# Drexubery/ViewCrafter

Measured on AMD Instinct MI355X. Metric: DDIM steps/sec (576x1024x25f latent 25x72x128, CFG 7.5, 50-step schedule), higher is better.
Workload: dtype f16; 1 GPU; ViewCrafter_25_576x1024x25; trajectories_per_gpu=1, frames=25, parallelism=trajectory-sharded x1 (no in-step collective)

## Files before the change

include/vcx.h:

```cpp
#ifndef VCX_H
#define VCX_H

#include <stddef.h>
#include <stdint.h>

#ifdef __cplusplus
extern "C" {
#endif

#define VCX_OK 0
#define VCX_EINVAL (-1)
#define VCX_ELAUNCH (-2)
#define VCX_ENODEV (-3)

#define VCX_ABI_VERSION 14

int vcx_abi_version(void);
const char* vcx_last_error(void);
int vcx_device_arch(char* name_host, int len);

#define VCX_GEMM_BIAS_N 0x1
#define VCX_GEMM_BIAS_M 0x2
#define VCX_GEMM_ROWADD 0x4
#define VCX_GEMM_RESIDUAL 0x8
#define VCX_GEMM_GEGLU 0x10
#define VCX_GEMM_OUT_F32 0x20
#define VCX_GEMM_CONV_SLABK 0x40
#define VCX_GEMM_LNFOLD 0x80
#define VCX_GEMM_LNFOLD_T 0x100
#define VCX_GEMM_COLSTATS 0x200
#define VCX_GEMM_ROWSTATS 0x400
#define VCX_GEMM_MXFP8_OUT 0x800

typedef struct vcx_gemm_desc {
    size_t struct_size;
    const void* A;
    const void* W;
    void* C;
    const float* bias;
    const float* rowadd;
    const void* residual;
    int64_t lda;
    int32_t M, N, K;
    int32_t ldw, ldc, ldr;
    int32_t mode;
    int32_t in_h, in_w, out_h, out_w, cin, kh, kw, stride, pad_h, pad_w, ups;
    int32_t rowadd_div;
    int32_t flags;
    float alpha;
    const float* ln_stats;
    const float* ln_colsum;
    float* colstats;
    int64_t ldcs;
    float* rowstats;
    float rowstats_eps;
    int32_t rowadd_ld;
    const void* tail_a0;
    const void* tail_a1;
    int64_t tail_lda0;
    int64_t tail_lda1;
    int32_t tail_k0;
    int32_t tail_k1;
} vcx_gemm_desc;

int vcx_gemm_f16(const vcx_gemm_desc* desc_host, void* stream);
int vcx_gemm_units_f16(const vcx_gemm_desc* desc_host, int unit_rows, int64_t w_unit_stride, int64_t bias_unit_stride, void* stream);

enum {
    VCX_ROUTE_REFUSED = 0,
    VCX_ROUTE_REGISTER = 1,
    VCX_ROUTE_TILED = 2,
    VCX_ROUTE_WS320 = 3,
    VCX_ROUTE_WS320_GEGLU = 4,
    VCX_ROUTE_WS320_LNF = 5,
    VCX_ROUTE_UNITS_WS320 = 6,
    VCX_ROUTE_UNITS_GROUPED = 7,
    VCX_ROUTE_UNITS_LOOP = 8
};
int vcx_gemm_route(const vcx_gemm_desc* desc_host, int unit_rows);

size_t vcx_groupnorm_ws_bytes(int n_outer, int64_t pixels, int groups);
int vcx_groupnorm_stats_f16(const void* x, float* stats, void* ws, int n_outer, int64_t pixels,
                            int C, int groups, void* stream);
int vcx_groupnorm_apply_f16(const void* x, void* y, const float* stats, const float* gamma,
                            const float* beta, int n_outer, int64_t pixels, int C, int groups,
                            float eps, int silu, void* stream);
int vcx_groupnorm_apply2_f16(const void* x1, int c1, const void* x2, void* y, const float* stats, const float* gamma, const float* beta,
                             int n_outer, int64_t pixels, int C, int groups, float eps, int silu, void* stream);
int vcx_groupnorm_stats_from_colstats_f32(const float* colstats, float* stats, void* ws, int n_outer, int64_t pixels, int C,
                                          int groups, void* stream);

int vcx_groupnorm_fold_linear_f16(const float* W, const float* bias, const float* gamma, const float* beta, const float* stats,
                                  void* Wn, float* bn, int n_outer, int N, int C, int groups, float eps, void* stream);

int vcx_rowstats_f16(const void* x, float* stats, int64_t rows, int C, float eps, void* stream);
int vcx_layernorm_f16(const void* x, void* y, const float* gamma, const float* beta,
                      int64_t rows, int C, float eps, void* stream);

int vcx_quant_mxfp8_f16(const void* x, int64_t ldx, void* q, void* scales, int64_t rows, int K, void* stream);
int vcx_layernorm_mxfp8_f16(const void* x, void* q, void* scales, const float* gamma, const float* beta, int64_t rows, int C, float eps,
                            void* stream);
int vcx_gemm_mxfp8(const void* a, const void* a_scales, const void* w, const void* w_scales, void* out, void* out_scales, const float* bias,
                   const void* residual, int64_t M, int64_t N, int64_t K, int64_t ldc, int64_t ldr, int flags, void* stream);
int vcx_gemm_mxfp8_ok(int64_t M, int64_t N, int64_t K, int flags);
int vcx_groupnorm_apply_mxfp8_f16(const void* x, void* q, void* scales, const float* stats, const float* gamma, const float* beta, int n_outer,
                                  int64_t pixels, int C, int groups, float eps, int silu, void* stream);
int vcx_conv_t3_mxfp8(const void* a, const void* a_scales, const void* w, const void* w_scales, void* out, const float* bias, const void* residual,
                      float* colstats, int64_t B, int64_t T, int64_t P, int64_t Cin, int64_t N, int64_t ldc, int64_t ldr, int64_t ldcs, int flags,
                      void* stream);
int vcx_conv_t3_mxfp8_ok(int64_t B, int64_t T, int64_t P, int64_t Cin, int64_t N, int64_t ldc, int64_t ldr, int64_t ldcs, int64_t colstats_col,
                         int flags);
int vcx_groupnorm_apply2_mxfp8_f16(const void* x1, int c1, const void* x2, void* q, void* scales, const float* stats, const float* gamma,
                                   const float* beta, int n_outer, int64_t pixels, int C, int groups, float eps, int silu, void* stream);
int vcx_conv3x3_mxfp8(const void* a, const void* a_scales, const void* w, const void* w_scales, void* out, const float* bias, const float* rowadd,
                      const void* residual, float* colstats, int64_t n, int64_t H, int64_t W, int64_t Cin, int64_t N, int64_t ldc, int64_t ldr,
                      int64_t ldcs, int64_t rowadd_ld, int64_t rowadd_div, int flags, void* stream);
int vcx_conv3x3_mxfp8_ok(int64_t n, int64_t H, int64_t W, int64_t Cin, int64_t N, int64_t ldc, int64_t ldr, int64_t ldcs, int64_t colstats_col,
                         int64_t rowadd_div, int flags);

#define VCX_ATTN_ACCUMULATE 1
#define VCX_ATTN_LOG2_LOGITS 2
int vcx_attn_flash_d64_f16(const void* q, const void* k, const void* vt, void* o, int n_groups,
                           int heads, int nq, int nk, int kv_rows, int kv_div, int64_t ldq,
                           int64_t ldk, int64_t ldvt, int64_t ldo, float scale, int flags,
                           void* stream);

int vcx_attn_flash_dual_d64_f16(const void* q, const void* k1, const void* vt1, const void* k2,
                                const void* vt2, void* o, int n_groups, int heads, int nq,
                                int nk1, int kv_rows1, int kv_div1, int64_t ldk1, int64_t ldvt1,
                                int nk2, int kv_rows2, int kv_div2, int64_t ldk2, int64_t ldvt2,
                                int64_t ldq, int64_t ldo, float scale, int flags, void* stream);

int vcx_attn_flash_d512_f16(const void* q, const void* k, const void* vt, void* o, int n_groups, int nq, int nk, int kv_rows,
                            int64_t ldq, int64_t ldk, int64_t ldvt, int64_t ldo, float scale, void* stream);

int vcx_attn_temporal_d64_f16(const void* qkv, void* o, int B, int T, int64_t P, int heads,
                              int64_t ld, int k_off, int v_off, int64_t ldo, float scale,
                              void* stream);
#define VCX_ATTN_CAUSAL 4
int vcx_attn_temporal_d64_masked_f16(const void* qkv, void* o, int B, int T, int64_t P, int heads,
                                     int64_t ld, int k_off, int v_off, int64_t ldo, float scale,
                                     int flags, void* stream);
int vcx_attn_temporal_d64_rel_f16(const void* qkv, void* o, const void* relg, void* relp, int R, int B, int T, int64_t P,
                                  int heads, int64_t ld, int k_off, int v_off, int64_t ldo, float scale, int flags,
                                  void* stream);

int vcx_softmax_rows_f16(void* x, int64_t rows, int n, int64_t ld, void* stream);

int vcx_silu_f32(const float* x, float* y, int64_t n, void* stream);
int vcx_gelu_f16(const void* x, void* y, int64_t n, void* stream);
int vcx_clip_preprocess_f32(const float* x, float* y, int B, int C, int H, int W, int size, int antialias,
                            const float* mean_host, const float* std_host, void* stream);
int vcx_timestep_embedding_f32(const int64_t* t, float* out, int B, int dim, float max_period,
                               void* stream);
int vcx_cast_f32_to_f16(const float* x, void* y, int64_t n, void* stream);
int vcx_cast_f16_to_f32(const void* x, float* y, int64_t n, void* stream);
int vcx_copy2d_f16(const void* src, void* dst, int64_t rows, int cols, int64_t lds, int64_t ldd,
                   void* stream);
int vcx_avgpool2x2_f16(const void* x, void* y, int n, int H, int W, int C, void* stream);
int vcx_upsample2x_f16(const void* x, void* y, int n, int H, int W, int C, void* stream);
int vcx_add_nchw_f32_to_nhwc_f16(const float* src, void* h, int n, int C, int64_t HW, void* stream);
int vcx_ncthw_f32_to_nthwc_f16(const float* src, void* dst, int B, int C, int T, int64_t HW,
                               int ldc, int c_off, float scale, void* stream);
int vcx_nthwc_to_ncthw_f32(const void* src, float* dst, int B, int C, int T, int64_t HW, int ldc,
                           int src_f32, void* stream);

size_t vcx_ddim_ws_bytes(int B, int64_t n);
int vcx_ddim_step_f32(const float* x, const float* v_cond, const float* v_uncond,
                      const float* noise, float* x_prev, float* pred_x0, void* ws,
                      size_t ws_bytes, int B, int64_t n, const float* coef_host, void* stream);
int vcx_ddim_step3_f32(const float* x, const float* v_cond, const float* v_uncond,
                       const float* v_img, const float* noise, float* x_prev, float* pred_x0,
                       void* ws, size_t ws_bytes, int B, int64_t n, const float* coef_host,
                       void* stream);

#define VCX_PROF_FAMILIES 6
int vcx_profile_begin(int max_records);
int vcx_profile_end(double* out_host);

#define VCX_TUNE_GEMM_CFG 0
#define VCX_TUNE_GEMM_DMA 1
#define VCX_TUNE_FLASH_QB 2
#define VCX_TUNE_XATTN_RESIDENT 3
#define VCX_TUNE_FLASH_IMPL 4
#define VCX_TUNE_EXP0 5
#define VCX_TUNE_EXP1 6
#define VCX_TUNE_GEMM_WS 7
#define VCX_TUNE_COUNT 8
int vcx_tune_set(int knob, int value);
int vcx_tune_get(int knob);

#ifdef __cplusplus
}
#endif
#endif
```

viewcrafter_amd/_lib.py:

```python
import ctypes
import os
from ctypes import c_char_p, c_double, c_float, c_int, c_int32, c_int64, c_void_p, POINTER

_HERE = os.path.dirname(os.path.abspath(__file__))
LIB_PATH = os.path.join(_HERE, "libvcx.so")

SYMBOLS = [
    "vcx_abi_version", "vcx_last_error", "vcx_device_arch", "vcx_gemm_f16", "vcx_gemm_units_f16", "vcx_gemm_route", "vcx_quant_mxfp8_f16", "vcx_layernorm_mxfp8_f16", "vcx_gemm_mxfp8", "vcx_gemm_mxfp8_ok",
    "vcx_groupnorm_apply_mxfp8_f16", "vcx_conv_t3_mxfp8", "vcx_conv_t3_mxfp8_ok",
    "vcx_groupnorm_apply2_mxfp8_f16", "vcx_conv3x3_mxfp8", "vcx_conv3x3_mxfp8_ok",
    "vcx_groupnorm_ws_bytes", "vcx_groupnorm_stats_f16", "vcx_groupnorm_apply_f16", "vcx_groupnorm_apply2_f16", "vcx_groupnorm_stats_from_colstats_f32", "vcx_groupnorm_fold_linear_f16", "vcx_layernorm_f16", "vcx_rowstats_f16",
    "vcx_attn_flash_d64_f16", "vcx_attn_flash_d512_f16", "vcx_attn_flash_dual_d64_f16", "vcx_attn_temporal_d64_f16", "vcx_attn_temporal_d64_masked_f16", "vcx_attn_temporal_d64_rel_f16", "vcx_softmax_rows_f16",
    "vcx_silu_f32", "vcx_gelu_f16", "vcx_clip_preprocess_f32", "vcx_add_nchw_f32_to_nhwc_f16", "vcx_timestep_embedding_f32", "vcx_cast_f32_to_f16", "vcx_cast_f16_to_f32",
    "vcx_copy2d_f16", "vcx_avgpool2x2_f16", "vcx_upsample2x_f16", "vcx_ncthw_f32_to_nthwc_f16", "vcx_nthwc_to_ncthw_f32", "vcx_ddim_ws_bytes", "vcx_ddim_step_f32", "vcx_ddim_step3_f32",
    "vcx_profile_begin", "vcx_profile_end", "vcx_tune_set", "vcx_tune_get",
]

ABI_VERSION = 14
TUNE = {"GEMM_CFG": (0, -1), "GEMM_DMA": (1, 1), "FLASH_QB": (2, 0), "XATTN_RESIDENT": (3, 1), "FLASH_IMPL": (4, 0), "EXP0": (5, 0),
        "EXP1": (6, 0), "GEMM_WS": (7, 1)}
GEMM_BIAS_N, GEMM_BIAS_M, GEMM_ROWADD, GEMM_RESIDUAL, GEMM_GEGLU, GEMM_OUT_F32, GEMM_CONV_SLABK = 1, 2, 4, 8, 16, 32, 64
GEMM_LNFOLD, GEMM_LNFOLD_T, GEMM_COLSTATS, GEMM_ROWSTATS, GEMM_MXFP8_OUT = 0x80, 0x100, 0x200, 0x400, 0x800
ROUTE_REFUSED, ROUTE_REGISTER, ROUTE_TILED, ROUTE_WS320, ROUTE_WS320_GEGLU, ROUTE_WS320_LNF, ROUTE_UNITS_WS320, ROUTE_UNITS_GROUPED, ROUTE_UNITS_LOOP = range(9)
PROF_FAMILIES = ("gemm", "flash_attn", "temporal_attn", "groupnorm", "layernorm", "elementwise")


class GemmDesc(ctypes.Structure):
    _fields_ = [
        ("struct_size", ctypes.c_size_t),
        ("A", c_void_p), ("W", c_void_p), ("C", c_void_p), ("bias", c_void_p), ("rowadd", c_void_p),
        ("residual", c_void_p), ("lda", c_int64), ("M", c_int32), ("N", c_int32), ("K", c_int32),
        ("ldw", c_int32), ("ldc", c_int32), ("ldr", c_int32), ("mode", c_int32),
        ("in_h", c_int32), ("in_w", c_int32), ("out_h", c_int32), ("out_w", c_int32), ("cin", c_int32),
        ("kh", c_int32), ("kw", c_int32), ("stride", c_int32), ("pad_h", c_int32), ("pad_w", c_int32),
        ("ups", c_int32), ("rowadd_div", c_int32), ("flags", c_int32), ("alpha", c_float),
        ("ln_stats", c_void_p), ("ln_colsum", c_void_p), ("colstats", c_void_p), ("ldcs", c_int64),
        ("rowstats", c_void_p), ("rowstats_eps", c_float), ("rowadd_ld", c_int32),
        ("tail_a0", c_void_p), ("tail_a1", c_void_p), ("tail_lda0", c_int64), ("tail_lda1", c_int64), ("tail_k0", c_int32), ("tail_k1", c_int32),
    ]

    def __init__(self, *args, **kw):
        super().__init__(*args, **kw)
        self.struct_size = ctypes.sizeof(GemmDesc)


_lib = None


class VcxError(RuntimeError):
    pass


def lib():
    global _lib
    if _lib is not None:
        return _lib
    if not os.path.exists(LIB_PATH):
        raise VcxError(
            f"{LIB_PATH} not found: build it with `make -C viewcrafter_amd/csrc` "
            "(or `python -c 'import __graft_entry__ as g; g.build()'`). There is no fallback path.")
    import torch
    L = ctypes.CDLL(LIB_PATH)
    L.vcx_abi_version.restype = c_int
    L.vcx_last_error.restype = c_char_p
    L.vcx_device_arch.argtypes = [c_char_p, c_int]
    L.vcx_gemm_f16.argtypes = [POINTER(GemmDesc), c_void_p]
    L.vcx_gemm_units_f16.argtypes = [POINTER(GemmDesc), c_int, c_int64, c_int64, c_void_p]
    L.vcx_gemm_route.argtypes = [POINTER(GemmDesc), c_int]
    L.vcx_quant_mxfp8_f16.argtypes = [c_void_p, c_int64, c_void_p, c_void_p, c_int64, c_int, c_void_p]
    L.vcx_layernorm_mxfp8_f16.argtypes = [c_void_p, c_void_p, c_void_p, c_void_p, c_void_p, c_int64, c_int, c_float, c_void_p]
    L.vcx_gemm_mxfp8.argtypes = [c_void_p, c_void_p, c_void_p, c_void_p, c_void_p, c_void_p, c_void_p, c_void_p, c_int64, c_int64, c_int64, c_int64,
                                 c_int64, c_int, c_void_p]
    L.vcx_gemm_mxfp8_ok.argtypes = [c_int64, c_int64, c_int64, c_int]
    L.vcx_groupnorm_apply_mxfp8_f16.argtypes = [c_void_p, c_void_p, c_void_p, c_void_p, c_void_p, c_void_p, c_int, c_int64, c_int, c_int, c_float, c_int, c_void_p]
    L.vcx_conv_t3_mxfp8.argtypes = [c_void_p, c_void_p, c_void_p, c_void_p, c_void_p, c_void_p, c_void_p, c_void_p, c_int64, c_int64, c_int64, c_int64, c_int64,
                                    c_int64, c_int64, c_int64, c_int, c_void_p]
    L.vcx_conv_t3_mxfp8_ok.argtypes = [c_int64, c_int64, c_int64, c_int64, c_int64, c_int64, c_int64, c_int64, c_int64, c_int]
    L.vcx_groupnorm_apply2_mxfp8_f16.argtypes = [c_void_p, c_int, c_void_p, c_void_p, c_void_p, c_void_p, c_void_p, c_void_p, c_int, c_int64, c_int, c_int, c_float,
                                                 c_int, c_void_p]
    L.vcx_conv3x3_mxfp8.argtypes = [c_void_p, c_void_p, c_void_p, c_void_p, c_void_p, c_void_p, c_void_p, c_void_p, c_void_p, c_int64, c_int64, c_int64, c_int64,
                                    c_int64, c_int64, c_int64, c_int64, c_int64, c_int64, c_int, c_void_p]
    L.vcx_conv3x3_mxfp8_ok.argtypes = [c_int64, c_int64, c_int64, c_int64, c_int64, c_int64, c_int64, c_int64, c_int64, c_int64, c_int]
    L.vcx_groupnorm_ws_bytes.argtypes = [c_int, c_int64, c_int]
    L.vcx_groupnorm_stats_f16.argtypes = [c_void_p, c_void_p, c_void_p, c_int, c_int64, c_int, c_int, c_void_p]
    L.vcx_groupnorm_apply_f16.argtypes = [c_void_p, c_void_p, c_void_p, c_void_p, c_void_p, c_int, c_int64, c_int,
                                          c_int, c_float, c_int, c_void_p]
    L.vcx_groupnorm_apply2_f16.argtypes = [c_void_p, c_int, c_void_p, c_void_p, c_void_p, c_void_p, c_void_p, c_int, c_int64, c_int,
                                           c_int, c_float, c_int, c_void_p]
    L.vcx_layernorm_f16.argtypes = [c_void_p, c_void_p, c_void_p, c_void_p, c_int64, c_int, c_float, c_void_p]
    L.vcx_rowstats_f16.argtypes = [c_void_p, c_void_p, c_int64, c_int, c_float, c_void_p]
    L.vcx_groupnorm_stats_from_colstats_f32.argtypes = [c_void_p, c_void_p, c_void_p, c_int, c_int64, c_int, c_int, c_void_p]
    L.vcx_groupnorm_fold_linear_f16.argtypes = [c_void_p, c_void_p, c_void_p, c_void_p, c_void_p, c_void_p, c_void_p, c_int, c_int, c_int, c_int,
                                                c_float, c_void_p]
    L.vcx_attn_flash_d64_f16.argtypes = [c_void_p, c_void_p, c_void_p, c_void_p, c_int, c_int, c_int, c_int, c_int,
                                         c_int, c_int64, c_int64, c_int64, c_int64, c_float, c_int, c_void_p]
    L.vcx_attn_flash_d512_f16.argtypes = [c_void_p, c_void_p, c_void_p, c_void_p, c_int, c_int, c_int, c_int, c_int64, c_int64, c_int64, c_int64, c_float, c_void_p]
    L.vcx_attn_flash_dual_d64_f16.argtypes = [c_void_p, c_void_p, c_void_p, c_void_p, c_void_p, c_void_p, c_int, c_int, c_int,
                                              c_int, c_int, c_int, c_int64, c_int64, c_int, c_int, c_int, c_int64, c_int64,
                                              c_int64, c_int64, c_float, c_int, c_void_p]
    L.vcx_attn_temporal_d64_f16.argtypes = [c_void_p, c_void_p, c_int, c_int, c_int64, c_int, c_int64, c_int, c_int,
                                            c_int64, c_float, c_void_p]
    L.vcx_attn_temporal_d64_masked_f16.argtypes = [c_void_p, c_void_p, c_int, c_int, c_int64, c_int, c_int64, c_int, c_int,
                                            c_int64, c_float, c_int, c_void_p]
    L.vcx_attn_temporal_d64_rel_f16.argtypes = [c_void_p, c_void_p, c_void_p, c_void_p, c_int, c_int, c_int, c_int64, c_int, c_int64, c_int, c_int,
                                                c_int64, c_float, c_int, c_void_p]
    L.vcx_softmax_rows_f16.argtypes = [c_void_p, c_int64, c_int, c_int64, c_void_p]
    L.vcx_silu_f32.argtypes = [c_void_p, c_void_p, c_int64, c_void_p]
    L.vcx_gelu_f16.argtypes = [c_void_p, c_void_p, c_int64, c_void_p]
    L.vcx_add_nchw_f32_to_nhwc_f16.argtypes = [c_void_p, c_void_p, c_int, c_int, c_int64, c_void_p]
    L.vcx_clip_preprocess_f32.argtypes = [c_void_p, c_void_p, c_int, c_int, c_int, c_int, c_int, c_int, POINTER(c_float), POINTER(c_float),
                                          c_void_p]
    L.vcx_timestep_embedding_f32.argtypes = [c_void_p, c_void_p, c_int, c_int, c_float, c_void_p]
    L.vcx_cast_f32_to_f16.argtypes = [c_void_p, c_void_p, c_int64, c_void_p]
    L.vcx_cast_f16_to_f32.argtypes = [c_void_p, c_void_p, c_int64, c_void_p]
    L.vcx_copy2d_f16.argtypes = [c_void_p, c_void_p, c_int64, c_int, c_int64, c_int64, c_void_p]
    L.vcx_avgpool2x2_f16.argtypes = [c_void_p, c_void_p, c_int, c_int, c_int, c_int, c_void_p]
    L.vcx_upsample2x_f16.argtypes = [c_void_p, c_void_p, c_int, c_int, c_int, c_int, c_void_p]
    L.vcx_ncthw_f32_to_nthwc_f16.argtypes = [c_void_p, c_void_p, c_int, c_int, c_int, c_int64, c_int, c_int, c_float,
                                             c_void_p]
    L.vcx_nthwc_to_ncthw_f32.argtypes = [c_void_p, c_void_p, c_int, c_int, c_int, c_int64, c_int, c_int, c_void_p]
    L.vcx_ddim_ws_bytes.restype = ctypes.c_size_t
    L.vcx_ddim_ws_bytes.argtypes = [c_int, c_int64]
    L.vcx_ddim_step_f32.argtypes = [c_void_p, c_void_p, c_void_p, c_void_p, c_void_p, c_void_p, c_void_p, ctypes.c_size_t, c_int,
                                    c_int64, POINTER(c_float), c_void_p]
    L.vcx_ddim_step3_f32.argtypes = [c_void_p, c_void_p, c_void_p, c_void_p, c_void_p, c_void_p, c_void_p, c_void_p, ctypes.c_size_t,
                                     c_int, c_int64, POINTER(c_float), c_void_p]
    L.vcx_profile_begin.argtypes = [c_int]
    L.vcx_profile_end.argtypes = [POINTER(c_double)]
    L.vcx_tune_set.argtypes = [c_int, c_int]
    L.vcx_tune_get.argtypes = [c_int]
    for name in SYMBOLS:
        fn = getattr(L, name)
        if name == "vcx_groupnorm_ws_bytes":
            fn.restype = ctypes.c_size_t
        elif name != "vcx_last_error":
            fn.restype = c_int
    if L.vcx_abi_version() != ABI_VERSION:
        raise VcxError(f"libvcx ABI version {L.vcx_abi_version()} != {ABI_VERSION}; rebuild the library (make -C viewcrafter_amd/csrc)")
    _lib = L
    return L


def check(rc, what=""):
    if rc != 0:
        msg = lib().vcx_last_error().decode("utf-8", "replace")
        raise VcxError(f"libvcx call failed ({rc}) {what}: {msg}")
```

viewcrafter_amd/lvdm/modules/networks/openaimodel3d.py:

```python
import os

import torch
from torch import nn

from .... import ops
from ....packing import pack_conv, pack_conv3x3_mxfp8, pack_conv_t3_mxfp8, pack_conv_ups_folded
from ..attention import PackedModule, SpatialTransformer, TemporalTransformer, _f16, _f32
from ..flow import CAT_SPLIT, GN_EPILOGUE_STATS, GN_STATS_LEVEL, CatTarget, Flow, out_kwargs as _out_kwargs

SKIP_FOLD = os.environ.get("VCX_SKIP_FOLD", "1") != "0"
EMB_BATCHED = os.environ.get("VCX_EMB_BATCHED", "1") != "0"
TCONV_MXFP8 = os.environ.get("VCX_TCONV_MXFP8", "0") == "1"
TCONV_MXFP8_SKIP_DIMS = frozenset(int(v) for v in os.environ.get("VCX_TCONV_MXFP8_SKIP_DIMS", "320").split(",") if v.strip())
RESCONV_MXFP8 = os.environ.get("VCX_RESCONV_MXFP8", "0") == "1"
RESCONV_MXFP8_SKIP_DIMS = frozenset(int(v) for v in os.environ.get("VCX_RESCONV_MXFP8_SKIP_DIMS", "").split(",") if v.strip())
RESCONV_MXFP8_KEEP_FOLD = os.environ.get("VCX_RESCONV_MXFP8_KEEP_FOLD", "0") == "1"

class TimestepBlock(nn.Module):
    """Marker: modules whose forward takes the timestep embedding (reference openaimodel3d.py:19-28)."""


class TimestepEmbedSequential(nn.Sequential, TimestepBlock):

    def forward(self, x, emb, context=None, batch_size=None, cfg_repeat=1, flow=None, x2=None):
# ... 587 lines not shown
            h = ops.linear(f_emb, *pk["fe"][0], out_f32=True)
            emb = ops.linear(ops.to_f16(ops.silu_f32(h)), *pk["fe"][1], out_f32=True, rowadd=emb, rowadd_div=1)
        return ops.to_f16(ops.silu_f32(emb))

    def forward(self, x, timesteps, context=None, features_adapter=None, fs=None, **kwargs):
        if self.use_hip_graph and features_adapter is None and torch.cuda.is_available() and not torch.cuda.is_current_stream_capturing():
            return self.forward_graphed(x, timesteps, context, fs, cfg_repeat=int(kwargs.get("cfg_repeat", 1) or 1))
        return self._forward(x, timesteps, context=context, features_adapter=features_adapter, fs=fs, **kwargs)

    def forward_graphed(self, x, timesteps, context, fs, cfg_repeat=1):
        parts = list(x) if isinstance(x, (list, tuple)) else [x]
        key = (tuple(tuple(p.shape) for p in parts), context.data_ptr(), context._version, tuple(context.shape),
               None if fs is None else tuple(fs.shape), cfg_repeat)
        ent = self._graphs.get(key)
        if ent is None:
            static = dict(parts=[p.detach().clone().float() for p in parts], t=timesteps.detach().clone(),
                          fs=None if fs is None else fs.detach().clone())
            with torch.no_grad():
                self._forward(static["parts"], static["t"], context=context, fs=static["fs"], cfg_repeat=cfg_repeat)
                torch.cuda.synchronize()
                graph = torch.cuda.CUDAGraph()
                with torch.cuda.graph(graph):
                    out = self._forward(static["parts"], static["t"], context=context, fs=static["fs"], cfg_repeat=cfg_repeat)
            if len(self._graphs) >= 4:
                self._graphs.clear()
            ent = self._graphs[key] = (graph, static, out, context, self._context_kv(context, static["parts"][0].shape[2]))
        graph, static, out = ent[:3]
        for dst, src in zip(static["parts"], parts):
            dst.copy_(src)
        static["t"].copy_(timesteps)
        if fs is not None:
            static["fs"].copy_(fs)
        graph.replay()
        return out

    def _forward(self, x, timesteps, context=None, features_adapter=None, fs=None, cfg_repeat=1, **kwargs):
        ops.require_gpu()
        parts = list(x) if isinstance(x, (list, tuple)) else [x]
        b, _, t, hh, ww = parts[0].shape
        device = parts[0].device
        cin = sum(p.shape[1] for p in parts)
        if cin != self.in_channels:
            raise ValueError(f"expected {self.in_channels} input channels, got {cin}")
        r = int(cfg_repeat or 1)
        if context.shape[0] != b * r:
            raise ValueError(f"context batch {context.shape[0]} != {b} videos x cfg_repeat {r}")
        pk = self.packed()
        emb = self._embed(pk, timesteps, fs, b, device)
        ckv = self._context_kv(context, t)
        rbs = self.resblocks()
        if EMB_BATCHED and all(o % 4 == 0 for o, _ in pk["emb_off"].values()):
            emb_all = ops.linear(emb, pk["emb_w"], pk["emb_b"], out_f32=True)
            if r > 1:
                n_all = emb_all.shape[1]
                emb_all = ops.repeat_rows(emb_all.view(torch.float16).view(b, 2 * n_all), r).view(torch.float32).view(r * b, n_all)
            for rb in rbs:
                o, n_e = pk["emb_off"][id(rb)]
                rb._emb_all = emb_all[:, o:o + n_e]
        try:
            return self._forward_body(parts, pk, emb, ckv, b, t, hh, ww, cin, r, device, features_adapter)
        finally:
            for rb in rbs:
                rb._emb_all = None

    def _forward_body(self, parts, pk, emb, ckv, b, t, hh, ww, cin, r, device, features_adapter):
        cur_b = b

        def replicate(a):
            n_, H_, W_, C_ = a.shape
            return ops.repeat_rows(a.view(n_ * H_ * W_, C_), r).view(r * n_, H_, W_, C_)

        h = torch.empty((b, t, hh, ww, cin), dtype=torch.float16, device=device)
        off = 0
        for p in parts:
            ops.ncthw_to_nthwc(p.float(), h, c_off=off)
            off += p.shape[1]
        h = h.view(b * t, hh, ww, cin)

        lvl2 = GN_STATS_LEVEL >= 2

        def replicate_cs(c):
            if c is None:
                return None
            strips, C_, _ = c.shape
            return ops.repeat_rows(c.view(torch.float16).view(strips, C_ * 4), r).view(torch.float32).view(r * strips, C_, 2)

        hs = []
        adapter_idx = 0
        cs = None
        for i, module in enumerate(self.input_blocks):
            flow = Flow(colstats=cs, want=lvl2)
            if i == 0:
                h = ops.conv2d(h, pk["w_in"], pk["b_in"], kh=3, kw=3)
                flow.colstats = None
                if self.addition_attention:
                    h = self.init_attn(h, emb, context=ckv, batch_size=cur_b, flow=flow)
            elif cur_b != b * r and any(isinstance(layer, SpatialTransformer) for layer in module):
                h = module(h, emb, context=ckv, batch_size=cur_b, cfg_repeat=r, flow=flow)
                cur_b = b * r
                emb = ops.repeat_rows(emb, r)
                hs = [(replicate(a), replicate_cs(c)) for a, c in hs]
            else:
                h = module(h, emb, context=ckv, batch_size=cur_b, flow=flow)
            cs = flow.colstats
            if features_adapter is not None and (i + 1) % 3 == 0:
                h = ops.add_nchw_(h.contiguous(), _adapter_rows(features_adapter[adapter_idx], h.shape[0]))
                adapter_idx, cs = adapter_idx + 1, None
            hs.append((h, cs))
        if features_adapter is not None and len(features_adapter) != adapter_idx:
            raise ValueError("Wrong features_adapter")
        if cur_b != b * r:
            h, cs, hs, emb, cur_b = replicate(h), replicate_cs(cs), [(replicate(a), replicate_cs(c)) for a, c in hs], ops.repeat_rows(emb, r), b * r
        b = cur_b
        if not lvl2:
            h = self.middle_block(h, emb, context=ckv, batch_size=b)
            for module in self.output_blocks:
                skip, _ = hs.pop()
                n, H, W, c1 = h.shape
                h = ops.concat_channels(h.view(n * H * W, c1), skip.view(n * H * W, skip.shape[-1])).view(n, H, W, -1)
                h = module(h, emb, context=ckv, batch_size=b)
            cs = None
        else:
            def target_for(n_, H_, W_, c_left, consumer):
                skip, skip_cs = hs[-1]
                M_ = n_ * H_ * W_
                ok = skip_cs is not None and ops.colstats_ok(M_, H_ * W_, 64, c_left + skip.shape[-1])
                split = CAT_SPLIT and SKIP_FOLD and c_left % 64 == 0 and skip.shape[-1] % 64 == 0 and isinstance(list(consumer)[0], ResBlock)
                return CatTarget(M_, c_left, skip.shape[-1], device, with_moments=ok, split=split)
            n, H, W, _ = h.shape
            tgt = target_for(n, H, W, _out_channels_of(self.middle_block), self.output_blocks[0])
            flow = Flow(colstats=cs, target=tgt)
            h = self.middle_block(h, emb, context=ckv, batch_size=b, flow=flow)
            for j, module in enumerate(self.output_blocks):
                skip, skip_cs = hs.pop()
                n, H, W, c1 = h.shape
                M, c2 = n * H * W, skip.shape[-1]
                if not tgt.split:
                    ops.copy2d(skip.view(M, c2), tgt.data[:, c1:], M, c2, c2, tgt.ld)
                if tgt.moments is not None:
                    ops.copy2d(skip_cs.view(torch.float16).view(M // 64, c2 * 4), tgt.moments.view(torch.float16).view(M // 64, tgt.ld * 4)[:, c1 * 4:],
                               M // 64, c2 * 4, c2 * 4, tgt.ld * 4)
                hcat, cat_cs = tgt.data.view(n, H, W, tgt.data_ld), tgt.moments
                x2 = skip if tgt.split else None
                tgt = None
                if j + 1 < len(self.output_blocks):
                    last = list(module)[-1]
                    up = 2 if isinstance(last, Upsample) or (isinstance(last, ResBlock) and last.up) else 1
                    tgt = target_for(n, H * up, W * up, _out_channels_of(module), self.output_blocks[j + 1])
                flow = Flow(colstats=cat_cs, want=tgt is None, target=tgt)
                h = module(hcat, emb, context=ckv, batch_size=b, flow=flow, x2=x2)
            cs = flow.colstats
        n, H, W, c = h.shape
        stats = None if cs is None else ops.group_norm_stats_from_colstats(cs, n, H * W, c)
        a = ops.group_norm(h.view(n, H * W, c), *pk["g_out"], True, stats=stats)
        y = ops.conv2d(a.view(n, H, W, c), pk["w_out"], pk["b_out"], kh=3, kw=3, out_f32=True)
        return ops.nthwc_to_ncthw(y.view(b, t, H, W, self.out_channels))
```

viewcrafter_amd/ops.py:

```python
import ctypes
import os

import torch

from ._lib import (GEMM_BIAS_M, GEMM_BIAS_N, GEMM_COLSTATS, GEMM_CONV_SLABK, GEMM_GEGLU, GEMM_LNFOLD, GEMM_LNFOLD_T, GEMM_MXFP8_OUT, GEMM_OUT_F32, GEMM_RESIDUAL, GEMM_ROWADD, GEMM_ROWSTATS, PROF_FAMILIES,
                   ROUTE_UNITS_GROUPED, ROUTE_UNITS_LOOP, ROUTE_UNITS_WS320, TUNE, GemmDesc, VcxError, check, lib)
from .packing import conv_slab_major

_f16 = torch.float16
_f32 = torch.float32
LN_ROWSTATS = os.environ.get("VCX_LN_ROWSTATS", "1") != "0"


def _stream():
    return torch.cuda.current_stream().cuda_stream


def _ptr(t):
    return t.data_ptr() if t is not None else None


def _dev16(*tensors):
    for t in tensors:
        if t is not None and (t.dtype is not _f16 or not t.is_cuda):
# ... 552 lines not shown
def flash_attn_d512(q, k, vt, out, *, n_groups, nq, nk, kv_rows, ldq, ldk, ldvt, ldo, scale):
    _dev16(q, k, vt, out)
    check(lib().vcx_attn_flash_d512_f16(q.data_ptr(), k.data_ptr(), vt.data_ptr(), out.data_ptr(), n_groups, nq, nk, kv_rows, ldq, ldk, ldvt, ldo,
                                        scale, _stream()), "attn_flash_d512")
    return out


def flash_attn_dual(q, k1, vt1, k2, vt2, out, *, n_groups, heads, nq, nk1, kv_rows1, kv_div1, ldk1, ldvt1, nk2, kv_rows2, kv_div2,
                    ldk2, ldvt2, ldq, ldo, scale, log2_logits=False):
    _dev16(q, k1, vt1, k2, vt2, out)
    check(lib().vcx_attn_flash_dual_d64_f16(q.data_ptr(), k1.data_ptr(), vt1.data_ptr(), k2.data_ptr(), vt2.data_ptr(),
                                            out.data_ptr(), n_groups, heads, nq, nk1, kv_rows1, kv_div1, ldk1, ldvt1, nk2,
                                            kv_rows2, kv_div2, ldk2, ldvt2, ldq, ldo, scale,
                                            ATTN_LOG2_LOGITS if log2_logits else 0, _stream()), "attn_flash_dual_d64")
    return out


def temporal_attn(qkv, out, *, B, T, P, heads, ld, k_off, v_off, ldo, scale, causal=False):
    _dev16(qkv, out)
    if causal:
        check(lib().vcx_attn_temporal_d64_masked_f16(qkv.data_ptr(), out.data_ptr(), B, T, P, heads, ld, k_off, v_off, ldo, scale, ATTN_CAUSAL,
                                                     _stream()), "attn_temporal_d64(causal)")
    else:
        check(lib().vcx_attn_temporal_d64_f16(qkv.data_ptr(), out.data_ptr(), B, T, P, heads, ld, k_off, v_off, ldo, scale,
                                              _stream()), "attn_temporal_d64")
    return out


def temporal_attn_rel(qkv, out, relg, relp, *, R, B, T, P, heads, ld, k_off, v_off, ldo, scale, causal=False):
    _dev16(qkv, out, relg, relp)
    check(lib().vcx_attn_temporal_d64_rel_f16(qkv.data_ptr(), out.data_ptr(), relg.data_ptr(), relp.data_ptr(), int(R), B, T, P, heads, ld, k_off, v_off,
                                              ldo, scale, ATTN_CAUSAL if causal else 0, _stream()), "attn_temporal_d64(rel)")
    return out


def softmax_rows_(x, n=None):
    rows = x.shape[0]
    check(lib().vcx_softmax_rows_f16(x.data_ptr(), rows, n if n is not None else x.shape[1], x.stride(0), _stream()),
          "softmax_rows")
    return x


def silu_f32(x):
    out = torch.empty_like(x)
    check(lib().vcx_silu_f32(x.data_ptr(), out.data_ptr(), x.numel(), _stream()), "silu")
    return out


def gelu_(x):
    check(lib().vcx_gelu_f16(x.data_ptr(), x.data_ptr(), x.numel(), _stream()), "gelu")
    return x


def clip_preprocess(x, size, antialias, mean, std):
    x = x.contiguous()
    _dev32(x)
    B, C, H, W = x.shape
    out = torch.empty((B, C, size, size), dtype=_f32, device=x.device)
    m = (ctypes.c_float * C)(*[float(v) for v in mean])
    s = (ctypes.c_float * C)(*[float(v) for v in std])
    check(lib().vcx_clip_preprocess_f32(x.data_ptr(), out.data_ptr(), B, C, H, W, int(size), 1 if antialias else 0, m, s, _stream()),
          "clip_preprocess")
    return out


def timestep_embedding(t, dim, max_period=10000.0):
    t = t.to(torch.int64).contiguous()
    out = torch.empty((t.shape[0], dim), dtype=_f32, device=t.device)
    check(lib().vcx_timestep_embedding_f32(t.data_ptr(), out.data_ptr(), t.shape[0], dim, max_period, _stream()),
          "timestep_embedding")
    return out


def to_f16(x):
    x = x.contiguous()
    out = torch.empty(x.shape, dtype=_f16, device=x.device)
    check(lib().vcx_cast_f32_to_f16(x.data_ptr(), out.data_ptr(), x.numel(), _stream()), "cast_f32_to_f16")
    return out


def to_f32(x):
    x = x.contiguous()
    out = torch.empty(x.shape, dtype=_f32, device=x.device)
    check(lib().vcx_cast_f16_to_f32(x.data_ptr(), out.data_ptr(), x.numel(), _stream()), "cast_f16_to_f32")
    return out


def copy2d(src, dst, rows, cols, lds, ldd):
    check(lib().vcx_copy2d_f16(src.data_ptr(), dst.data_ptr(), rows, cols, lds, ldd, _stream()), "copy2d")


def avgpool2x2(x):
    n, H, W, C = x.shape
    x = x.contiguous()
    out = torch.empty((n, H // 2, W // 2, C), dtype=_f16, device=x.device)
    check(lib().vcx_avgpool2x2_f16(x.data_ptr(), out.data_ptr(), n, H, W, C, _stream()), "avgpool2x2")
    return out


def upsample2x(x):
    n, H, W, C = x.shape
    x = x.contiguous()
    out = torch.empty((n, 2 * H, 2 * W, C), dtype=_f16, device=x.device)
    check(lib().vcx_upsample2x_f16(x.data_ptr(), out.data_ptr(), n, H, W, C, _stream()), "upsample2x")
    return out


def repeat_rows(x, r):
    rows, C = x.shape
    out = torch.empty((r * rows, C), dtype=x.dtype, device=x.device)
    assert x.dtype == _f16
    for i in range(r):
        copy2d(x, out[i * rows:], rows, C, x.stride(0), C)
    return out


def concat_channels(a, b):
    rows, ca = a.shape
    cb = b.shape[1]
    out = torch.empty((rows, ca + cb), dtype=_f16, device=a.device)
    copy2d(a, out, rows, ca, a.stride(0), ca + cb)
    copy2d(b, out[:, ca:], rows, cb, b.stride(0), ca + cb)
    return out


def add_nchw_(h, feat):
    n, H, W, C = h.shape
    feat = feat.float().contiguous()
    if tuple(feat.shape) != (n, C, H, W):
        raise VcxError(f"adapter feature {tuple(feat.shape)} does not match the activation [{n}, {C}, {H}, {W}]")
    _dev16(h)
    _dev32(feat)
    check(lib().vcx_add_nchw_f32_to_nhwc_f16(feat.data_ptr(), h.data_ptr(), n, C, H * W, _stream()), "add_nchw")
    return h


def ncthw_to_nthwc(src, dst, c_off=0, scale=1.0):
    B, C, T, H, W = src.shape
    src = src.contiguous()
    check(lib().vcx_ncthw_f32_to_nthwc_f16(src.data_ptr(), dst.data_ptr(), B, C, T, H * W, dst.shape[-1], c_off, scale,
                                           _stream()), "ncthw_to_nthwc")
    return dst


def nthwc_to_ncthw(src, C=None):
    B, T, H, W, ldc = src.shape
    C = ldc if C is None else C
    out = torch.empty((B, C, T, H, W), dtype=_f32, device=src.device)
    check(lib().vcx_nthwc_to_ncthw_f32(src.data_ptr(), out.data_ptr(), B, C, T, H * W, ldc,
                                       1 if src.dtype == _f32 else 0, _stream()), "nthwc_to_ncthw")
    return out


def ddim_step(x, v_cond, v_uncond, noise, coef, ws=None, v_img=None, cfg_img=0.0):
    B = x.shape[0]
    n = x.numel() // B
    x_prev = torch.empty_like(x)
    pred_x0 = torch.empty_like(x)
    if ws is None:
        ws = torch.empty((lib().vcx_ddim_ws_bytes(B, n) // 8,), dtype=torch.float64, device=x.device)
    c = (ctypes.c_float * 9)(*([float(v) for v in coef[:8]] + [float(cfg_img)]))
    check(lib().vcx_ddim_step3_f32(x.data_ptr(), v_cond.data_ptr(), _ptr(v_uncond), _ptr(v_img), _ptr(noise),
                                   x_prev.data_ptr(), pred_x0.data_ptr(), ws.data_ptr(), ws.numel() * ws.element_size(), B, n, c,
                                   _stream()), "ddim_step")
    return x_prev, pred_x0


def tune_set(name, value):
    return lib().vcx_tune_set(TUNE[name][0], int(value))


def tune_get(name):
    return lib().vcx_tune_get(TUNE[name][0])


def tune_report():
    return {k: tune_get(k) for k, (_, d) in TUNE.items() if tune_get(k) != d}


def profile_begin(max_records=1 << 16):
    check(lib().vcx_profile_begin(max_records), "profile_begin")


def profile_end():
    buf = (ctypes.c_double * (4 * len(PROF_FAMILIES)))()
    check(lib().vcx_profile_end(buf), "profile_end")
    out = {}
    for i, name in enumerate(PROF_FAMILIES):
        out[name] = dict(launches=int(buf[4 * i]), ms=buf[4 * i + 1], flops=buf[4 * i + 2], bytes=buf[4 * i + 3])
    return out
```

Before: 5.869 DDIM steps/s.

## Fuse UNet output GroupNorm+SiLU, 3x3 conv and NCTHW transpose into one kernel

Adds a single HIP kernel for the UNet output head. It applies GroupNorm and SiLU to halo tiles as they are staged into LDS, then runs the 3x3 conv to the few output channels with MFMA and writes f32 directly in NCTHW layout. This removes the normalized f16 intermediate, the separate conv launch and the layout-transpose pass. The price is a padded-N MFMA (16 lanes for at most 8 output channels) and halo recomputation of the norm, and it is gated by shape checks and an env flag.

```diff
diff --git a/include/vcx.h b/include/vcx.h
--- a/include/vcx.h
+++ b/include/vcx.h
@@ -13,7 +13,7 @@
 #define VCX_ELAUNCH (-2)
 #define VCX_ENODEV (-3)
 
-#define VCX_ABI_VERSION 14
+#define VCX_ABI_VERSION 15
 
 int vcx_abi_version(void);
 const char* vcx_last_error(void);
@@ -90,6 +90,11 @@
 int vcx_groupnorm_stats_from_colstats_f32(const float* colstats, float* stats, void* ws, int n_outer, int64_t pixels, int C,
                                           int groups, void* stream);
 
+int vcx_unet_out_f32(const void* h, int64_t ld, const float* stats, const float* gamma, const float* beta, float eps, const void* w,
+                     const float* bias, float* out, int64_t n, int64_t T, int64_t H, int64_t W, int64_t C, int64_t cout, int64_t groups,
+                     void* stream);
+int vcx_unet_out_ok(int64_t n, int64_t T, int64_t H, int64_t W, int64_t C, int64_t cout, int64_t ld, int64_t groups);
+
 int vcx_groupnorm_fold_linear_f16(const float* W, const float* bias, const float* gamma, const float* beta, const float* stats,
                                   void* Wn, float* bn, int n_outer, int N, int C, int groups, float eps, void* stream);
 
diff --git a/viewcrafter_amd/_lib.py b/viewcrafter_amd/_lib.py
--- a/viewcrafter_amd/_lib.py
+++ b/viewcrafter_amd/_lib.py
@@ -9,14 +9,14 @@
     "vcx_abi_version", "vcx_last_error", "vcx_device_arch", "vcx_gemm_f16", "vcx_gemm_units_f16", "vcx_gemm_route", "vcx_quant_mxfp8_f16", "vcx_layernorm_mxfp8_f16", "vcx_gemm_mxfp8", "vcx_gemm_mxfp8_ok",
     "vcx_groupnorm_apply_mxfp8_f16", "vcx_conv_t3_mxfp8", "vcx_conv_t3_mxfp8_ok",
     "vcx_groupnorm_apply2_mxfp8_f16", "vcx_conv3x3_mxfp8", "vcx_conv3x3_mxfp8_ok",
-    "vcx_groupnorm_ws_bytes", "vcx_groupnorm_stats_f16", "vcx_groupnorm_apply_f16", "vcx_groupnorm_apply2_f16", "vcx_groupnorm_stats_from_colstats_f32", "vcx_groupnorm_fold_linear_f16", "vcx_layernorm_f16", "vcx_rowstats_f16",
+    "vcx_groupnorm_ws_bytes", "vcx_groupnorm_stats_f16", "vcx_groupnorm_apply_f16", "vcx_groupnorm_apply2_f16", "vcx_groupnorm_stats_from_colstats_f32", "vcx_unet_out_f32", "vcx_unet_out_ok", "vcx_groupnorm_fold_linear_f16", "vcx_layernorm_f16", "vcx_rowstats_f16",
     "vcx_attn_flash_d64_f16", "vcx_attn_flash_d512_f16", "vcx_attn_flash_dual_d64_f16", "vcx_attn_temporal_d64_f16", "vcx_attn_temporal_d64_masked_f16", "vcx_attn_temporal_d64_rel_f16", "vcx_softmax_rows_f16",
     "vcx_silu_f32", "vcx_gelu_f16", "vcx_clip_preprocess_f32", "vcx_add_nchw_f32_to_nhwc_f16", "vcx_timestep_embedding_f32", "vcx_cast_f32_to_f16", "vcx_cast_f16_to_f32",
     "vcx_copy2d_f16", "vcx_avgpool2x2_f16", "vcx_upsample2x_f16", "vcx_ncthw_f32_to_nthwc_f16", "vcx_nthwc_to_ncthw_f32", "vcx_ddim_ws_bytes", "vcx_ddim_step_f32", "vcx_ddim_step3_f32",
     "vcx_profile_begin", "vcx_profile_end", "vcx_tune_set", "vcx_tune_get",
 ]
 
-ABI_VERSION = 14
+ABI_VERSION = 15
 TUNE = {"GEMM_CFG": (0, -1), "GEMM_DMA": (1, 1), "FLASH_QB": (2, 0), "XATTN_RESIDENT": (3, 1), "FLASH_IMPL": (4, 0), "EXP0": (5, 0),
         "EXP1": (6, 0), "GEMM_WS": (7, 1)}
 GEMM_BIAS_N, GEMM_BIAS_M, GEMM_ROWADD, GEMM_RESIDUAL, GEMM_GEGLU, GEMM_OUT_F32, GEMM_CONV_SLABK = 1, 2, 4, 8, 16, 32, 64
@@ -92,6 +92,9 @@
     L.vcx_groupnorm_stats_from_colstats_f32.argtypes = [c_void_p, c_void_p, c_void_p, c_int, c_int64, c_int, c_int, c_void_p]
     L.vcx_groupnorm_fold_linear_f16.argtypes = [c_void_p, c_void_p, c_void_p, c_void_p, c_void_p, c_void_p, c_void_p, c_int, c_int, c_int, c_int,
                                                 c_float, c_void_p]
+    L.vcx_unet_out_f32.argtypes = [c_void_p, c_int64, c_void_p, c_void_p, c_void_p, c_float, c_void_p, c_void_p, c_void_p, c_int64, c_int64, c_int64, c_int64,
+                                   c_int64, c_int64, c_int64, c_void_p]
+    L.vcx_unet_out_ok.argtypes = [c_int64] * 8
     L.vcx_attn_flash_d64_f16.argtypes = [c_void_p, c_void_p, c_void_p, c_void_p, c_int, c_int, c_int, c_int, c_int,
                                          c_int, c_int64, c_int64, c_int64, c_int64, c_float, c_int, c_void_p]
     L.vcx_attn_flash_d512_f16.argtypes = [c_void_p, c_void_p, c_void_p, c_void_p, c_int, c_int, c_int, c_int, c_int64, c_int64, c_int64, c_int64, c_float, c_void_p]
diff --git a/viewcrafter_amd/csrc/out_head.hip b/viewcrafter_amd/csrc/out_head.hip
--- /dev/null
+++ b/viewcrafter_amd/csrc/out_head.hip
@@ -0,0 +1,184 @@
+#include "vcx_common.h"
+
+namespace {
+
+constexpr int OH_PH = 8, OH_PW = 32;
+constexpr int OH_HH = OH_PH + 2, OH_HW = OH_PW + 2;
+constexpr int OH_NPIX = OH_HH * OH_HW;
+constexpr int OH_ITEMS = OH_NPIX * 8;
+constexpr int OH_THREADS = 256;
+constexpr int OH_IT = (OH_ITEMS + OH_THREADS - 1) / OH_THREADS;
+constexpr int OH_MAXCOUT = 8;
+
+__device__ __forceinline__ int oh_lds_off(int pix, int hx, int chunk) { return pix * 64 + ((chunk ^ ((hx >> 1) & 7)) << 3); }
+
+__global__ void __launch_bounds__(OH_THREADS, 2) unet_out_kernel(const half_t* __restrict__ x, int64_t ld, const float* __restrict__ stats,
+                                                                 const float* __restrict__ gamma, const float* __restrict__ beta,
+                                                                 const half_t* __restrict__ w, const float* __restrict__ bias,
+                                                                 float* __restrict__ out, int T, int H, int W, int C, int cout, float eps,
+                                                                 int tiles_x, int vec_store) {
+    __shared__ __attribute__((aligned(16))) half_t img[OH_NPIX * 64];
+    __shared__ float smean[32], srstd[32];
+    const int tid = threadIdx.x, n = blockIdx.y;
+    const int ty = blockIdx.x / tiles_x, tx = blockIdx.x - ty * tiles_x;
+    const int y0 = ty * OH_PH, x0 = tx * OH_PW;
+    const int cpg = C >> 5;
+    if (tid < 32) {
+        smean[tid] = stats[((int64_t)n * 32 + tid) * 2 + 0];
+        srstd[tid] = rsqrtf(stats[((int64_t)n * 32 + tid) * 2 + 1] + eps);
+    }
+
+    const half_t* xf = x + (int64_t)n * H * W * ld + (tid & 7) * 8;
+    int goff[OH_IT];
+    unsigned inside = 0;
+#pragma unroll
+    for (int k = 0; k < OH_IT; ++k) {
+        const int pix = (tid + k * OH_THREADS) >> 3;
+        const int hy = pix / OH_HW, hx = pix - hy * OH_HW;
+        const int iy = y0 - 1 + hy, ix = x0 - 1 + hx;
+        const bool in = pix < OH_NPIX && iy >= 0 && iy < H && ix >= 0 && ix < W;
+        goff[k] = in ? (int)((iy * W + ix) * ld) : 0;
+        inside |= (in ? 1u : 0u) << k;
+    }
+    const bool last_piece = tid + (OH_IT - 1) * OH_THREADS < OH_ITEMS;
+    h8 raw[OH_IT];
+    auto load_slab = [&](int s, bool real) {
+#pragma unroll
+        for (int k = 0; k < OH_IT; ++k) raw[k] = *reinterpret_cast<const h8*>(xf + (real ? goff[k] + s * 64 : 0));
+    };
+
+    const int wave = tid >> 6, lane = tid & 63;
+    const int lr = lane & 15, lg = lane >> 4;
+    bool active[4];
+    int apix[4], acol[4];
+#pragma unroll
+    for (int g = 0; g < 4; ++g) {
+        const int prow = 2 * wave + (g >> 1), pcol = (g & 1) * 16;
+        active[g] = y0 + prow < H && x0 + pcol < W;
+        apix[g] = prow * OH_HW + pcol + lr;
+        acol[g] = pcol + lr;
+    }
+    f4 acc[4];
+#pragma unroll
+    for (int g = 0; g < 4; ++g) acc[g] = f4{0.f, 0.f, 0.f, 0.f};
+    const half_t* wrow = w + (int64_t)min(lr, cout - 1) * 9 * C + lg * 8;
+
+    const int nslab = C >> 6;
+    load_slab(0, true);
+    __syncthreads();
+    for (int s = 0; s < nslab; ++s) {
+        h8 bf[9][2];
+#pragma unroll
+        for (int tap = 0; tap < 9; ++tap)
+#pragma unroll
+            for (int kk = 0; kk < 2; ++kk) {
+                const h8 v = *reinterpret_cast<const h8*>(wrow + (s * 9 + tap) * 64 + kk * 32);
+                bf[tap][kk] = lr < cout ? v : h8{0, 0, 0, 0, 0, 0, 0, 0};
+            }
+        float sc[8], mn[8], bt[8];
+#pragma unroll
+        for (int e = 0; e < 8; ++e) {
+            const int c = s * 64 + (tid & 7) * 8 + e;
+            const int g = c / cpg;
+            sc[e] = srstd[g] * gamma[c];
+            mn[e] = smean[g];
+            bt[e] = beta[c];
+        }
+#pragma unroll
+        for (int k = 0; k < OH_IT; ++k) {
+#pragma unroll
+            for (int e = 0; e < 8; ++e) {
+                float f = __builtin_fmaf((float)raw[k][e] - mn[e], sc[e], bt[e]);
+                f = vcx_silu(f);
+                raw[k][e] = (inside >> k) & 1 ? (half_t)f : (half_t)0.f;
+            }
+        }
+        static_assert(OH_IT == 11, "the operand lists below name every piece");
+        asm volatile("" : "+v"(raw[0]), "+v"(raw[1]), "+v"(raw[2]), "+v"(raw[3]), "+v"(raw[4]), "+v"(raw[5]), "+v"(raw[6]), "+v"(raw[7]), "+v"(raw[8]),
+                     "+v"(raw[9]), "+v"(raw[10]));
+#pragma unroll
+        for (int k = 0; k < OH_IT; ++k) {
+            const int pix = (tid + k * OH_THREADS) >> 3;
+            if (k < OH_IT - 1 || last_piece) *reinterpret_cast<h8*>(img + oh_lds_off(pix, pix % OH_HW, tid & 7)) = raw[k];
+        }
+        asm volatile("s_nop 1" : : "v"(raw[0]), "v"(raw[1]), "v"(raw[2]), "v"(raw[3]), "v"(raw[4]), "v"(raw[5]), "v"(raw[6]), "v"(raw[7]), "v"(raw[8]),
+                     "v"(raw[9]), "v"(raw[10]) : "memory");
+        load_slab(s + 1, s + 1 < nslab);
+        __syncthreads();
+#pragma unroll
+        for (int tap = 0; tap < 9; ++tap) {
+            const int tofs = (tap / 3) * OH_HW + tap % 3;
+            h8 a[2][4];
+#pragma unroll
+            for (int kk = 0; kk < 2; ++kk)
+#pragma unroll
+                for (int g = 0; g < 4; ++g) a[kk][g] = *reinterpret_cast<const h8*>(img + oh_lds_off(apix[g] + tofs, acol[g] + tap % 3, kk * 4 + lg));
+#pragma unroll
+            for (int kk = 0; kk < 2; ++kk)
+#pragma unroll
+                for (int g = 0; g < 4; ++g) acc[g] = __builtin_amdgcn_mfma_f32_16x16x32_f16(a[kk][g], bf[tap][kk], acc[g], 0, 0, 0);
+        }
+        __syncthreads();
+    }
+
+    if (lr < cout) {
+        const float bv = bias[lr];
+        const int bi = n / T, ti = n - bi * T;
+        float* oc = out + (((int64_t)bi * cout + lr) * T + ti) * H * W;
+#pragma unroll
+        for (int g = 0; g < 4; ++g) {
+            const int yy = y0 + 2 * wave + (g >> 1), xx = x0 + (g & 1) * 16 + lg * 4;
+            if (!active[g] || xx >= W) continue;
+            float* o = oc + (int64_t)yy * W + xx;
+            const f4 r = acc[g] + bv;
+            if (vec_store && xx + 3 < W) {
+                *reinterpret_cast<f4*>(o) = r;
+            } else {
+#pragma unroll
+                for (int e = 0; e < 4; ++e)
+                    if (xx + e < W) o[e] = r[e];
+            }
+        }
+    }
+}
+
+int unet_out_shape_ok(int64_t n, int64_t T, int64_t H, int64_t W, int64_t C, int64_t cout, int64_t ld, int64_t groups) {
+    auto no = [&](const char* why) {
+        vcx_set_error("vcx_unet_out_f32: %s (n=%lld T=%lld H=%lld W=%lld C=%lld cout=%lld ld=%lld groups=%lld)", why, (long long)n, (long long)T,
+                      (long long)H, (long long)W, (long long)C, (long long)cout, (long long)ld, (long long)groups);
+        return 0;
+    };
+    if (n <= 0 || T <= 0 || H <= 0 || W <= 0 || C <= 0 || cout <= 0) return no("every extent must be positive");
+    if (groups != 32) return no("32 groups only");
+    if (C % 64 != 0) return no("need C % 64 == 0");
+    if (cout > OH_MAXCOUT) return no("at most 8 output channels");
+    if (n % T != 0) return no("n must be a whole number of videos of T frames");
+    if (ld < C || ld % 8 != 0) return no("need a pixel stride ld >= C, ld % 8 == 0");
+    if (n > 65535) return no("at most 65535 frames");
+    if (H >= (1 << 24) || W >= (1 << 24) || H * W * ld >= ((int64_t)1 << 31)) return no("a frame must span fewer than 2^31 elements");
+    if (((H + OH_PH - 1) / OH_PH) * ((W + OH_PW - 1) / OH_PW) >= ((int64_t)1 << 31)) return no("too many patches per frame");
+    if (9 * C * cout >= ((int64_t)1 << 31)) return no("weight too large");
+    return 1;
+}
+
+}
+
+extern "C" int vcx_unet_out_ok(int64_t n, int64_t T, int64_t H, int64_t W, int64_t C, int64_t cout, int64_t ld, int64_t groups) {
+    return unet_out_shape_ok(n, T, H, W, C, cout, ld, groups);
+}
+
+extern "C" int vcx_unet_out_f32(const void* h, int64_t ld, const float* stats, const float* gamma, const float* beta, float eps, const void* w,
+                                const float* bias, float* out, int64_t n, int64_t T, int64_t H, int64_t W, int64_t C, int64_t cout, int64_t groups,
+                                void* stream) {
+    if (!unet_out_shape_ok(n, T, H, W, C, cout, ld, groups)) return VCX_EINVAL;
+    VCX_REQUIRE(h && stats && gamma && beta && w && bias && out, "vcx_unet_out_f32: null pointer");
+    VCX_REQUIRE((((uintptr_t)h | (uintptr_t)w) & 15) == 0 && ((uintptr_t)out & 3) == 0, "vcx_unet_out_f32: h / w must be 16-byte, out 4-byte aligned");
+    hipStream_t s = (hipStream_t)stream;
+    const double px = (double)n * H * W;
+    VcxProfScope prof(VCX_FAM_GEMM, s, 2.0 * px * cout * 9.0 * C, 2.0 * px * C + 4.0 * px * cout);
+    const int tiles_x = (int)((W + OH_PW - 1) / OH_PW), tiles_y = (int)((H + OH_PH - 1) / OH_PH);
+    const int vec_store = (W % 4 == 0) && (((uintptr_t)out & 15) == 0);
+    hipLaunchKernelGGL(unet_out_kernel, dim3((unsigned)(tiles_x * tiles_y), (unsigned)n), dim3(OH_THREADS), 0, s, (const half_t*)h, ld, stats, gamma, beta,
+                       (const half_t*)w, bias, out, (int)T, (int)H, (int)W, (int)C, (int)cout, eps, tiles_x, vec_store);
+    return vcx_check_launch("vcx_unet_out_f32");
+}
diff --git a/viewcrafter_amd/lvdm/modules/networks/openaimodel3d.py b/viewcrafter_amd/lvdm/modules/networks/openaimodel3d.py
--- a/viewcrafter_amd/lvdm/modules/networks/openaimodel3d.py
+++ b/viewcrafter_amd/lvdm/modules/networks/openaimodel3d.py
@@ -763,6 +763,10 @@
             cs = flow.colstats
         n, H, W, c = h.shape
         stats = None if cs is None else ops.group_norm_stats_from_colstats(cs, n, H * W, c)
+        if h.is_cuda and h.is_contiguous() and self.out[0].num_groups == 32 and ops.unet_out_ok(n, t, H, W, c, self.out_channels):
+            if stats is None:
+                stats = ops.group_norm_stats(h.view(n, H * W, c))
+            return ops.unet_out(h, stats, *pk["g_out"], pk["w_out"], pk["b_out"], frames=t)
         a = ops.group_norm(h.view(n, H * W, c), *pk["g_out"], True, stats=stats)
         y = ops.conv2d(a.view(n, H, W, c), pk["w_out"], pk["b_out"], kh=3, kw=3, out_f32=True)
         return ops.nthwc_to_ncthw(y.view(b, t, H, W, self.out_channels))
diff --git a/viewcrafter_amd/ops.py b/viewcrafter_amd/ops.py
--- a/viewcrafter_amd/ops.py
+++ b/viewcrafter_amd/ops.py
@@ -728,6 +728,35 @@
     return out
 
 
+OUT_FUSED = os.environ.get("VCX_OUT_FUSED", "1") != "0"
+
+
+def unet_out_ok(n, frames, H, W, C, cout, *, ld=None, groups=32):
+    if not OUT_FUSED:
+        return False
+    return lib().vcx_unet_out_ok(n, frames, H, W, C, cout, C if ld is None else ld, groups) == 1
+
+
+def unet_out(h, stats, gamma, beta, eps, w, bias, *, frames, groups=32):
+    _dev16(h, w)
+    _dev32(stats, gamma, beta, bias)
+    n, H, W, C = h.shape
+    ld = h.stride(2)
+    cout = w.shape[0]
+    if h.stride(3) != 1 or h.stride(1) != W * ld or h.stride(0) != H * W * ld:
+        raise VcxError(f"unet_out: h must be [n, H, W, C] with dense pixels of stride ld >= C, got strides {h.stride()}")
+    if w.dim() != 2 or w.shape[1] != 9 * C or not w.is_contiguous() or tuple(bias.shape) != (cout,):
+        raise VcxError(f"unet_out: weights must be contiguous [cout, 9 * {C}] with a [cout] bias, got {tuple(w.shape)} / {tuple(bias.shape)}")
+    if tuple(stats.shape) != (n, groups, 2) or not stats.is_contiguous() or gamma.numel() != C or beta.numel() != C:
+        raise VcxError(f"unet_out: statistics [n = {n}, {groups}, 2] and {C} affine parameters expected, got {tuple(stats.shape)} / {gamma.numel()}")
+    if frames <= 0 or n % frames != 0:
+        raise VcxError(f"unet_out: {n} frames are no whole number of videos of {frames}")
+    out = torch.empty((n // frames, cout, frames, H, W), dtype=_f32, device=h.device)
+    check(lib().vcx_unet_out_f32(h.data_ptr(), ld, stats.data_ptr(), gamma.data_ptr(), beta.data_ptr(), eps, w.data_ptr(), bias.data_ptr(),
+                                 out.data_ptr(), n, frames, H, W, C, cout, groups, _stream()), "unet_out")
+    return out
+
+
 def ddim_step(x, v_cond, v_uncond, noise, coef, ws=None, v_img=None, cfg_img=0.0):
     B = x.shape[0]
     n = x.numel() // B
```

Measured after the change: 5.881 DDIM steps/s (median of 6 runs). No clear change (+0.2%).
